# KubiakJakub01/Blokus-RL

Measured on AMD Instinct MI355X. Metric: MCTS sims/sec on 20x20 Blokus (4 players, 256 games/GPU, 100 sims/move), higher is better.
Workload: dtype fp32 net (fp32 operands split into f16 hi+lo, 3 f16 MFMA products, f32 accumulation: fp32-class error, tests/test_leafnet_gpu.py) / f64 search / u32 bitboards; 1 GPU; config 3 (N=1) / 4 (N=8): AlphaZero self-play 20x20, 256 concurrent games per GPU, 100 sims/move, ResNet-5x64 leaf eval; global_batch=256, parallelism=dp1 (independent games), model=resnet

## Files before the change

### blokus_rl_amd/csrc/mcts.hip

```cpp
#define BK_BOARD_SYNC() ::bk::wave_lds_sync()
#ifdef BK_STAMPS
#include <hip/hip_runtime.h>
static __device__ unsigned long long g_step_stamps[4096][16];
#define BK_MASK_STAMP(i) \
  do { if (threadIdx.x == 0 && blockIdx.x < 4096 && blockDim.x > 256) g_step_stamps[blockIdx.x][i] = __builtin_amdgcn_s_memtime(); } while (0)
#endif
#include <algorithm>
#include <cmath>
#include <cstring>
#include <vector>

#include "../../include/blokus_engine.h"
#include "ctx.h"
#include "legal_rows.h"
#include "mcts_dev.h"

namespace bk {

constexpr int kResetBlocks = 8;
__global__ __launch_bounds__(256) void k_reset(DevMcts m, const int32_t* flags) {
  const int t = blockIdx.y;
  if (flags && !flags[t]) return;
  TabEntry* tab = m.tab + (size_t)t * m.TS;
  for (int i = blockIdx.x * 256 + threadIdx.x; i < m.TS; i += kResetBlocks * 256) tab[i] = TabEntry{0ull, 0u, 0};
  if (blockIdx.x == 0 && threadIdx.x == 0) { m.tree_nodes[t] = 0; m.tree_children[t] = 0; }
}

constexpr int kSelectWaves = 4;
__global__ __launch_bounds__(64 * kSelectWaves) void k_select(DevPreset dp, DevMcts m, const uint32_t* __restrict__ roots,
                                                              const int32_t* __restrict__ active, double cpuct,
                                                              int32_t* __restrict__ status_out, float* __restrict__ obs,
                                                              uint64_t* __restrict__ mask_out, double root_eps, int t0) {
  extern __shared__ __attribute__((aligned(16))) uint32_t lds[];
  __shared__ int status_sh;
  const int t = t0 + blockIdx.x;
  const int wave = __builtin_amdgcn_readfirstlane(threadIdx.x >> 6);
  if (wave == 0) {
    const int st = select_descend(dp, m, t, roots, active, cpuct, status_out, lds, 0, nullptr, root_eps);
    if (lane_id() == 0) status_sh = st;
  }
  __syncthreads();
  select_leaf<kSelectWaves>(dp, m, t, status_sh, obs, mask_out, lds, wave);
}

constexpr int kLeafR = 1;
__global__ __launch_bounds__(256) void k_leaf_logits(DevPreset dp, DevMcts m, const float* __restrict__ feat,
                                                     int64_t ldf, int F, const float* __restrict__ W,
                                                     const float* __restrict__ bias) {
  extern __shared__ __attribute__((aligned(16))) uint32_t lds[];
  leaf_logits_tree<kLeafR>(dp, m, blockIdx.x, blockIdx.y, kLeafBlocks, feat, ldf, F, W, bias, lds);
}

__global__ __launch_bounds__(64) void k_expand_backup(DevPreset dp, DevMcts m, const float* __restrict__ logp,
                                                      const float* __restrict__ values, int prior_mode) {
  extern __shared__ __attribute__((aligned(16))) uint32_t lds[];
  expand_tree(dp, m, blockIdx.x, logp, values, prior_mode, lds);
}

__device__ __forceinline__ void wg_store_handoff() {
  __builtin_amdgcn_s_waitcnt(0x0F70);
  __syncthreads();
  asm volatile("buffer_inv sc0" ::: "memory");
}
constexpr int kStepWaves = 16;
__device__ __forceinline__ void leaf_zero_logits_tree(const DevPreset& dp, const DevMcts& m, int t,
                                                      const float* __restrict__ feat, int64_t ldf, int F,
                                                      uint32_t* lds) {
  const int K = leaf_logits_prologue(dp, m, t, 0, feat, ldf, F, lds);
  if (K < 0 || K > kLeafCap) return;
  const int32_t* ids = reinterpret_cast<const int32_t*>(lds + dp.W32pad);
  for (int j = threadIdx.x; j < K; j += blockDim.x) {
    m.leaf_ids[(size_t)t * kLeafCap + j] = ids[j];
    m.leaf_logit[(size_t)t * kLeafCap + j] = 0.0f;
  }
}
template <bool ROWS>
__device__ __forceinline__ void leaf_step_body(const DevPreset& dp, const DevMcts& m, const int t,
                                               const float* __restrict__ feat, int64_t ldf, int F,
                                               const float* __restrict__ W, const float* __restrict__ bias,
                                               const float* __restrict__ values, int do_select,
                                               const uint32_t* __restrict__ roots,
                                               const int32_t* __restrict__ active, double cpuct,
                                               int32_t* __restrict__ status_out, float* __restrict__ obs,
                                               uint64_t* __restrict__ mask_out, bool uninformed, int root_row) {
  extern __shared__ __attribute__((aligned(16))) uint32_t lds[];
  __shared__ int status_sh;
  const int wave = __builtin_amdgcn_readfirstlane(threadIdx.x >> 6);
#ifdef BK_STAMPS
#define BK_STEP_STAMP(i) \
  do { if (do_select && threadIdx.x == 0 && t < 4096) g_step_stamps[t][i] = __builtin_amdgcn_s_memtime(); } while (0)
#else
#define BK_STEP_STAMP(i) do { } while (0)
#endif
  BK_STEP_STAMP(0);
  if (ROWS && uninformed)
    leaf_zero_logits_tree(dp, m, t, feat, ldf, F, lds);
  else
    leaf_logits_tree<kLeafR>(dp, m, t, 0, 1, feat, ldf, F, W, bias, lds);
  wg_store_handoff();
  BK_STEP_STAMP(1);
  if (wave == 0) expand_tree<ROWS>(dp, m, t, nullptr, values, 2, lds);
  wg_store_handoff();
  BK_STEP_STAMP(2);
  if (!do_select) return;
  if (wave == 0) {
    const int st = select_descend<ROWS>(dp, m, t, roots, active, cpuct, status_out, lds, 0, nullptr, 1e-6, root_row);
    if (lane_id() == 0) status_sh = st;
  }
  __syncthreads();
  BK_STEP_STAMP(3);
  select_leaf<kStepWaves>(dp, m, t, status_sh, obs, mask_out, lds, wave);
  BK_STEP_STAMP(4);
#undef BK_STEP_STAMP
}
__global__ __launch_bounds__(64 * kStepWaves) void k_leaf_step(DevPreset dp, DevMcts m, const float* __restrict__ feat,
                                                                 int64_t ldf, int F, const float* __restrict__ W,
                                                                 const float* __restrict__ bias,
                                                                 const float* __restrict__ values, int do_select,
                                                                 const uint32_t* __restrict__ roots,
                                                                 const int32_t* __restrict__ active, double cpuct,
                                                                 int32_t* __restrict__ status_out,
                                                                 float* __restrict__ obs,
                                                                 uint64_t* __restrict__ mask_out, int t0) {
  leaf_step_body<false>(dp, m, t0 + blockIdx.x, feat, ldf, F, W, bias, values, do_select, roots, active, cpuct,
                        status_out, obs, mask_out, false, -1);
}

template <bool ROWS>
__device__ __forceinline__ void leaf_step_ov_body(const DevPreset& dp, const DevMcts& m, const int t,
                                                  const float* __restrict__ feat, int64_t ldf, int F,
                                                  const float* __restrict__ W, const float* __restrict__ bias,
                                                  const float* __restrict__ values, int do_select,
                                                  const uint32_t* __restrict__ roots,
                                                  const int32_t* __restrict__ active, double cpuct,
                                                  int32_t* __restrict__ status_out, float* __restrict__ obs,
                                                  uint64_t* __restrict__ mask_out, int sel_off, int skipz,
                                                  bool uninformed, int root_row) {
  extern __shared__ __attribute__((aligned(16))) uint32_t lds[];
  __shared__ int status_sh, status0_sh;
  __shared__ StepExpand sx;
  const int wave = __builtin_amdgcn_readfirstlane(threadIdx.x >> 6);
#ifdef BK_STAMPS
#define BK_OV_STAMP(i) \
  do { if (lane_id() == 0 && do_select && t < 4096) g_step_stamps[t][i] = __builtin_amdgcn_s_memtime(); } while (0)
#else
#define BK_OV_STAMP(i) do { } while (0)
#endif
  if (threadIdx.x == 0) {
    sx.ready = 0;
    sx.pready = 0;
    sx.done = 0;
    sx.leaf_ready = 0;
    sx.slice = 0;
    sx.loaded = 0;
    sx.counted = 0;
    sx.written = 0;
    sx.kready = 0;
    sx.hready = 0;
    status_sh = 0;
    status0_sh = m.leaf_status[t];
  }
  if (wave == 0) BK_OV_STAMP(0);
  LeafPre pre{0ull, 0.0f, false};
  if (wave > 0) pre = leaf_pre_load<kStepWaves - 1>(dp, m, t, feat, ldf, F);
  __syncthreads();
  const int status0 = status0_sh;
  int K = -1;
  if (wave > 0) {
    K = leaf_logits_prologue_w<kStepWaves - 1>(dp, m, t, feat, ldf, F, lds, wave, &sx, status0, &pre);
    if (wave == 1 && K >= 0) {
      wait_flag_acquire(&sx.hready);
      StepHead h;
      h.status = sx.hd_status;
      h.node = sx.hd_node;
      h.used = sx.hd_used;
      h.key = sx.hd_key;
      expand_head(m, t, h, K, &sx);
      BK_OV_STAMP(1);
    }
  }
  const int32_t* ids = reinterpret_cast<const int32_t*>(lds + dp.W32pad);
  float* lg = reinterpret_cast<float*>(lds + dp.W32pad + kLeafCap + F);
  uint32_t* lsel = lds + sel_off;
  uint32_t* m32 = lsel + kStateWords + 2 * kMaxN;
  if (wave == 0) {
    const StepHead h = backup_first<ROWS>(m, t, dp.P, values, status0);
    if (h.status == 1) {
      if (lane_id() == 0) {
        sx.hd_status = h.status;
        sx.hd_node = h.node;
        sx.hd_used = h.used;
        sx.hd_key = h.key;
        __hip_atomic_store(&sx.hready, 1, __ATOMIC_RELEASE, __HIP_MEMORY_SCOPE_WORKGROUP);
      }
    } else if (lane_id() == 0) {
      sx.err = -1;
      __hip_atomic_store(&sx.ready, 1, __ATOMIC_RELEASE, __HIP_MEMORY_SCOPE_WORKGROUP);
    }
    BK_OV_STAMP(2);
    if (do_select) {
      __builtin_amdgcn_s_waitcnt(0x0F70);
      asm volatile("buffer_inv sc0" ::: "memory");
      int* pend[3];
      pend[0] = &sx.ready;
      pend[1] = &sx.pready;
      pend[2] = &sx.err;
      const int st = select_descend<ROWS>(dp, m, t, roots, active, cpuct, status_out, lsel, h.key,
                                          h.status == 1 ? pend : nullptr, 1e-6, root_row);
      if (st == 1)
        for (int i = lane_id(); i < dp.W32pad / 4; i += kWave) reinterpret_cast<uint4*>(m32)[i] = make_uint4(0u, 0u, 0u, 0u);
      if (lane_id() == 0) {
        status_sh = st;
        __hip_atomic_store(&sx.leaf_ready, 1, __ATOMIC_RELEASE, __HIP_MEMORY_SCOPE_WORKGROUP);
      }
      BK_OV_STAMP(3);
      leaf_obs_rows<1>(dp, m, t, st, obs, lsel, lane_id());
    }
  }
  if (wave > 0 && K >= 0 && K <= kLeafCap) {
    if (ROWS && uninformed) {
      for (int j = (wave - 1) * kWave + lane_id(); j < K; j += (kStepWaves - 1) * kWave) lg[j] = 0.0f;
    } else {
      leaf_logits_dots<kLeafR>(dp, 0, K, wave - 1, kStepWaves - 1, W, bias, F, lds, nullptr, lg, skipz);
    }
    int done = 0;
    if (lane_id() == 0) done = __hip_atomic_fetch_add(&sx.done, 1, __ATOMIC_ACQ_REL, __HIP_MEMORY_SCOPE_WORKGROUP);
    done = readlane_i(done, 0);
    if (done == kStepWaves - 2) {
      BK_OV_STAMP(4);
      while (__hip_atomic_load(&sx.ready, __ATOMIC_ACQUIRE, __HIP_MEMORY_SCOPE_WORKGROUP) == 0)
        __builtin_amdgcn_s_sleep(1);
      const int err = readlane_i(sx.err, 0);
      if (err == 0) expand_children_lds(m, (int64_t)sx.off, K, ids, lg);
      BK_OV_STAMP(9);
      const bool descended = readlane_i(__hip_atomic_load(&sx.leaf_ready, __ATOMIC_RELAXED,
                                                          __HIP_MEMORY_SCOPE_WORKGROUP), 0) != 0;
      if (!descended) {
        __builtin_amdgcn_s_waitcnt(0x0F70);
        if (lane_id() == 0) __hip_atomic_store(&sx.pready, 1, __ATOMIC_RELEASE, __HIP_MEMORY_SCOPE_WORKGROUP);
      } else if (lane_id() == 0) {
        __hip_atomic_store(&sx.pready, 1, __ATOMIC_RELAXED, __HIP_MEMORY_SCOPE_WORKGROUP);
      }
      BK_OV_STAMP(5);
    }
  }
  if (do_select) {
    while (__hip_atomic_load(&sx.leaf_ready, __ATOMIC_ACQUIRE, __HIP_MEMORY_SCOPE_WORKGROUP) == 0)
      __builtin_amdgcn_s_sleep(1);
    if (readlane_i(status_sh, 0) == 1) mask_slices_claim(dp, lsel, m32, &sx.slice);
    if (wave == 0) BK_OV_STAMP(8);
  }
  __syncthreads();
  if (wave == 0) BK_OV_STAMP(6);
  if (!do_select) return;
  select_leaf<kStepWaves, true, false>(dp, m, t, status_sh, obs, mask_out, lsel, wave);
  if (wave == 0) BK_OV_STAMP(7);
#undef BK_OV_STAMP
}
__global__ __launch_bounds__(64 * kStepWaves) void k_leaf_step_ov(DevPreset dp, DevMcts m, const float* __restrict__ feat,
                                                                    int64_t ldf, int F, const float* __restrict__ W,
                                                                    const float* __restrict__ bias,
                                                                    const float* __restrict__ values, int do_select,
                                                                    const uint32_t* __restrict__ roots,
                                                                    const int32_t* __restrict__ active, double cpuct,
                                                                    int32_t* __restrict__ status_out,
                                                                    float* __restrict__ obs,
                                                                    uint64_t* __restrict__ mask_out, int sel_off,
                                                                    int skipz, int t0) {
  leaf_step_ov_body<false>(dp, m, t0 + blockIdx.x, feat, ldf, F, W, bias, values, do_select, roots, active, cpuct,
                           status_out, obs, mask_out, sel_off, skipz, false, -1);
}

struct RowTabs {
  const int32_t *tree, *net, *sims;
};
struct RowHeads {
  const float* W[BK_ARENA_MAX_NETS];
  const float* bias[BK_ARENA_MAX_NETS];
  int n;
};
__device__ __forceinline__ int row_live_tree(const RowTabs& rows, int r, int sim, int& budget) {
  const int t = __builtin_amdgcn_readfirstlane(rows.tree[r]);
  budget = 0;
  if (t < 0) return -1;
  budget = __builtin_amdgcn_readfirstlane(rows.sims[r]);
  return sim < budget ? t : -1;
}
__device__ __forceinline__ bool row_head(const RowTabs& rows, const RowHeads& hd, int r, const float*& W,
                                         const float*& bias, bool& uninformed) {
  const int k = __builtin_amdgcn_readfirstlane(rows.net[r]);
  uninformed = k < 0;
  W = k == 0 ? hd.W[0] : k == 1 ? hd.W[1] : k == 2 ? hd.W[2] : k == 3 ? hd.W[3] : nullptr;
  bias = k == 0 ? hd.bias[0] : k == 1 ? hd.bias[1] : k == 2 ? hd.bias[2] : k == 3 ? hd.bias[3] : nullptr;
  return k < hd.n;
}

__global__ __launch_bounds__(64 * kSelectWaves) void k_select_rows(DevPreset dp, DevMcts m, RowTabs rows,
                                                                   const uint32_t* __restrict__ roots, double cpuct,
                                                                   int32_t* __restrict__ status_out) {
  extern __shared__ __attribute__((aligned(16))) uint32_t lds[];
  __shared__ int status_sh;
  int budget;
  const int t = row_live_tree(rows, blockIdx.x, 0, budget);
  if (t < 0 || t >= m.T) return;
  const int wave = __builtin_amdgcn_readfirstlane(threadIdx.x >> 6);
  if (wave == 0) {
    const int st = select_descend<true>(dp, m, t, roots, nullptr, cpuct, status_out, lds, 0, nullptr, 1e-6, (int)blockIdx.x);
    if (lane_id() == 0) status_sh = st;
  }
  __syncthreads();
  select_leaf<kSelectWaves>(dp, m, t, status_sh, nullptr, nullptr, lds, wave);
}

__global__ __launch_bounds__(64 * kStepWaves) void k_leaf_step_rows(DevPreset dp, DevMcts m, RowTabs rows, int sim,
                                                                      const float* __restrict__ feat, int64_t ldf, int F,
                                                                      RowHeads heads, const float* __restrict__ values,
                                                                      int do_select, const uint32_t* __restrict__ roots,
                                                                      double cpuct, int32_t* __restrict__ status_out) {
  int budget;
  const int t = row_live_tree(rows, blockIdx.x, sim, budget);
  if (t < 0 || t >= m.T) return;
  const float *W, *bias;
  bool uninformed;
  if (!row_head(rows, heads, blockIdx.x, W, bias, uninformed)) return;
  leaf_step_body<true>(dp, m, t, feat, ldf, F, W, bias, uninformed ? nullptr : values,
                       do_select && sim + 1 < budget, roots, nullptr, cpuct, status_out, nullptr, nullptr, uninformed,
                       (int)blockIdx.x);
}

__global__ __launch_bounds__(64 * kStepWaves) void k_leaf_step_ov_rows(DevPreset dp, DevMcts m, RowTabs rows, int sim,
                                                                         const float* __restrict__ feat, int64_t ldf,
                                                                         int F, RowHeads heads,
                                                                         const float* __restrict__ values, int do_select,
                                                                         const uint32_t* __restrict__ roots, double cpuct,
                                                                         int32_t* __restrict__ status_out, int sel_off,
                                                                         int skipz) {
  int budget;
  const int t = row_live_tree(rows, blockIdx.x, sim, budget);
  if (t < 0 || t >= m.T) return;
  const float *W, *bias;
  bool uninformed;
  if (!row_head(rows, heads, blockIdx.x, W, bias, uninformed)) return;
  leaf_step_ov_body<true>(dp, m, t, feat, ldf, F, W, bias, uninformed ? nullptr : values,
                          do_select && sim + 1 < budget, roots, nullptr, cpuct, status_out, nullptr, nullptr, sel_off,
                          skipz, uninformed, (int)blockIdx.x);
}

__global__ __launch_bounds__(64) void k_arena_move(DevMcts m, RowTabs rows, const uint32_t* __restrict__ roots,
                                                   int32_t* __restrict__ action) {
  const int r = blockIdx.x, l = lane_id();
  const int t = __builtin_amdgcn_readfirstlane(rows.tree[r]);
  if (t < 0 || t >= m.T) {
    if (l == 0) action[r] = -1;
    return;
  }
  const uint64_t key = table_key(roots + (size_t)r * kStateWords);
  int64_t off;
  int K;
  if (!table_find(m, t, key, off, K, nullptr)) {
    if (l == 0) {
      action[r] = -1;
      atomicOr(&m.counters[kCtrErr], (unsigned long long)kErrMissingRoot);
    }
    return;
  }
  double best = -1.0;
  int bi = 0x7fffffff;
  for (int i = l; i < K; i += kWave) {
    const double v = (double)m.ch_N[off + i];
    if (v > best) { best = v; bi = i; }
  }
  wave_argmax(best, bi);
  if (l == 0) action[r] = K > 0 ? m.ch_id[off + bi] : -1;
}

__device__ __forceinline__ double raise_visits(uint32_t n, double e) {
  if (e == 1.0 || n <= 1u) return (double)n;
  return pow((double)n, e);
}

__global__ __launch_bounds__(64) void k_root(DevMcts m, const uint32_t* __restrict__ roots,
                                             const int32_t* __restrict__ active, double temperature, int mode,
                                             int32_t* ids, double* pi, uint32_t* n_out, double* q_out, float* p_out,
                                             int cap, int32_t* counts) {
  const int t = blockIdx.x;
  const int l = lane_id();
  if (active && !active[t]) {
    if (l == 0) counts[t] = 0;
    return;
  }
  const uint32_t* s = roots + (size_t)t * kStateWords;
  const uint64_t key = table_key(s);
  int64_t off;
  int K;
  if (!table_find(m, t, key, off, K, nullptr)) {
    if (l == 0) { counts[t] = -1; atomicOr(&m.counters[kCtrErr], (unsigned long long)kErrMissingRoot); }
    return;
  }
  if (l == 0) counts[t] = K <= cap ? K : -K;
  const int Kc = K <= cap ? K : cap;
  if (mode == 1) {
    for (int i = l; i < Kc; i += kWave) {
      ids[(size_t)t * cap + i] = m.ch_id[off + i];
      n_out[(size_t)t * cap + i] = m.ch_N[off + i];
      q_out[(size_t)t * cap + i] = m.ch_Q[off + i];
      p_out[(size_t)t * cap + i] = m.ch_P[off + i];
    }
    return;
  }
// ... 502 lines not shown
```

### blokus_rl_amd/csrc/mcts_dev.h

```cpp
#pragma once
#include <cmath>
#include <vector>

#include "../../include/blokus_engine.h"
#include "ctx.h"
#include "legal_rows.h"

namespace bk {

constexpr int kMaxDepth = 96;
constexpr int kExpandLdsIds = 2048;
constexpr int kGatherRegs = 16;
constexpr int kLeafCap = 2048;
constexpr int kLeafBlocks = 4;
constexpr int kMaxFeat = 2048;
constexpr int kLeafQ = 16;

#ifdef BK_STAMPS
static __device__ unsigned long long g_stamps[2][4096][8];
#define BK_STAMP(k, i) \
  do { if (lane_id() == 0 && blockIdx.x < 4096) g_stamps[k][blockIdx.x][i] = __builtin_amdgcn_s_memtime(); } while (0)
#else
#define BK_STAMP(k, i) do { } while (0)
#endif
// ... 139 lines not shown
    const double sq = sqrt((double)(uint32_t)wave_sum((int)vs) + eps);
    for (int i = l; i < K; i += kWave) {
      const double h = Q[i] + ((cp * (double)P[i]) * sq) / (1.0 + (double)Nn[i]);
      if (h > best) { best = h; bi = i; bid = ID[i]; }
    }
  }
  wave_argmax(best, bi);
  id_out = readlane_i(bid, bi & (kWave - 1));
  return bi;
}

__device__ __forceinline__ void wait_flag_acquire(int* flag) {
  while (__hip_atomic_load(flag, __ATOMIC_ACQUIRE, __HIP_MEMORY_SCOPE_WORKGROUP) == 0) __builtin_amdgcn_s_sleep(1);
  asm volatile("buffer_inv sc0" ::: "memory");
}
template <bool ROOT_ROW = false>
__device__ __forceinline__ int select_descend(const DevPreset& dp, const DevMcts& m, int t,
                                              const uint32_t* __restrict__ roots, const int32_t* __restrict__ active,
                                              double cpuct, int32_t* __restrict__ status_out, uint32_t* lds,
                                              uint64_t pend_key = 0, int* const* pend = nullptr,
                                              double root_eps = 1e-6, int root_row = -1) {
  uint32_t* s = lds;
  uint64_t* fa = reinterpret_cast<uint64_t*>(lds + kStateWords);
  const int l = lane_id();
  if (active && !active[t]) {
    if (l == 0) {
      m.leaf_status[t] = 0;
      if (status_out) status_out[t] = 0;
      m.depth[t] = 0;
    }
    return 0;
  }
  BK_STAMP(0, 0);
  load_state(s, roots + (size_t)(ROOT_ROW ? root_row : t) * kStateWords);
  BK_BOARD_SYNC();
  BK_STAMP(0, 1);
  double cp = cpuct, eps = root_eps;
  int depth = 0, err = 0;
  long long scanned = 0;
  int64_t rec_child = 0;
  int rec_pl = 0;
#ifdef BK_STAMPS
  unsigned long long t_probe = 0, t_child = 0, t_apply = 0, t_adv = 0;
#define BK_TACC(v, stmt)                                         \
  do {                                                           \
    const unsigned long long t0_ = __builtin_amdgcn_s_memtime(); \
    stmt;                                                        \
    v += __builtin_amdgcn_s_memtime() - t0_;                     \
  } while (0)
#else
#define BK_TACC(v, stmt) \
  do {                   \
    stmt;                \
  } while (0)
#endif
  for (;;) {
    int64_t off;
    int Kn;
    bool found;
    const uint64_t key = table_key(s);
    int* pend_children = nullptr;
    if (pend && key == pend_key) {
      wait_flag_acquire(pend[0]);
      if (readlane_i(*pend[2], 0) == 0) pend_children = pend[1];
      pend = nullptr;
    }
    BK_TACC(t_probe, found = table_find(m, t, key, off, Kn, nullptr));
    if (!found) break;
    if (Kn <= 0) { err |= kErrIllegal; break; }
    if (pend_children) wait_flag_acquire(pend_children);
    scanned += Kn;
    int a, ci;
    BK_TACC(t_child, ci = select_child(m, off, Kn, cp, a, eps));
    if (ci < 0 || ci >= Kn) { err |= kErrIllegal; break; }
    if (depth >= kMaxDepth) { err |= kErrDepth; break; }
    const int p = (int)s[kWToMove];
    int bad;
    BK_TACC(t_apply, bad = place_action<false>(dp, s, a, fa));
    BK_TACC(t_adv, if (!bad) advance_turn(dp, s, p, [&](int q) { return rows_any_legal(dp, s, q); }));
    if (bad) { err |= kErrIllegal; break; }
    if (depth < kWave) {
      if (l == depth) {
        rec_child = off + ci;
        rec_pl = (int)s[kWToMove];
      }
    } else if (l == 0) {
      const size_t pi = (size_t)t * kMaxDepth + depth;
      m.path_child[pi] = off + ci;
      m.path_pl[pi] = (int)s[kWToMove];
    }
    ++depth;
    cp = 1.0;
    eps = 1e-6;
  }
  if (l < depth && l < kWave) {
    const size_t pi = (size_t)t * kMaxDepth + l;
    m.path_child[pi] = rec_child;
    m.path_pl[pi] = rec_pl;
  }
  BK_STAMP(0, 2);
#ifdef BK_STAMPS
  if (lane_id() == 0 && blockIdx.x < 4096) {
    g_stamps[0][blockIdx.x][6] = t_probe;
    g_stamps[0][blockIdx.x][7] = t_child;
    g_stamps[1][blockIdx.x][7] = t_apply;
    g_stamps[1][blockIdx.x][6] = t_adv;
  }
#endif
#undef BK_TACC
  int status;
  if (err) {
    status = 0;
  } else if (s[kWFlags] & kFlagOver) {
    status = 2;
    if (l == 0) terminal_scores(dp, s, m.leaf_scores + (size_t)t * kMaxP);
  } else {
    status = 1;
  }
  if (l == 0) {
    m.leaf_status[t] = status;
    if (status_out) status_out[t] = status;
    m.depth[t] = depth;
    ctr_add(m, t, kCtrLevels, (unsigned long long)depth);
    ctr_add(m, t, kCtrScanned, (unsigned long long)scanned);
    if (status == 2) ctr_add(m, t, kCtrTerminal, 1ull);
    if (err) atomicOr(&m.counters[kCtrErr], (unsigned long long)err);
  }
  return status;
}

template <int NW>
__device__ __forceinline__ void leaf_obs_rows(const DevPreset& dp, const DevMcts& m, int t, int status,
                                              float* __restrict__ obs, const uint32_t* s, int tid) {
  if (status == 1 && tid < kWave) store_state(m.leaf_state + (size_t)t * kStateWords, s);
  const int obs_len = 2 * dp.P * dp.N * dp.N;
  float* o = obs ? obs + (size_t)t * obs_len : nullptr;
  const int tm = (int)s[kWToMove];
  const int rows = 2 * dp.P * dp.N;
  for (int pr = tid; o && pr < rows; pr += NW * kWave) {
    const int plane = pr / dp.N, r = pr - plane * dp.N;
    uint32_t bits = 0u;
    if (status == 1) bits = plane < dp.P ? s[plane * kMaxN + r] : ((plane - dp.P) == tm ? dp.full_row : 0u);
    float* dst = o + pr * dp.N;
    if ((dp.N & 3) == 0) {
      for (int c = 0; c < dp.N; c += 4)
        *reinterpret_cast<float4*>(dst + c) = make_float4((float)((bits >> c) & 1u), (float)((bits >> (c + 1)) & 1u),
                                                          (float)((bits >> (c + 2)) & 1u), (float)((bits >> (c + 3)) & 1u));
    } else {
      for (int c = 0; c < dp.N; ++c) dst[c] = (float)((bits >> c) & 1u);
    }
  }
}

template <int NW, bool BUILT = false, bool OBS = true>
__device__ __forceinline__ void select_leaf(const DevPreset& dp, const DevMcts& m, int t, int status,
                                            float* __restrict__ obs, uint64_t* __restrict__ mask_out, uint32_t* lds,
                                            int wave) {
  const uint32_t* s = lds;
  uint32_t* m32 = lds + kStateWords + 2 * kMaxN;
  const int l = lane_id(), tid = wave * kWave + l;
  const int obs_len = 2 * dp.P * dp.N * dp.N;
  if (status == 1) {
    if (BUILT)
      ;
    else if (NW == 1)
      build_mask_rows(dp, s, (int)s[kWToMove], m32);
    else
      build_mask_rows_wg<(NW > kMaskWpb ? kMaskWpb : NW)>(dp, s, (int)s[kWToMove], m32, wave);
    BK_STAMP(0, 3);
    uint64_t* mo = m.leaf_mask + (size_t)t * dp.W64;
    uint64_t* mo2 = mask_out ? mask_out + (size_t)t * dp.W64 : nullptr;
    for (int j = tid; j < dp.W64; j += NW * kWave) {
      const uint64_t w = (uint64_t)m32[2 * j] | ((uint64_t)m32[2 * j + 1] << 32);
      mo[j] = w;
      if (mo2) mo2[j] = w;
    }
    if (wave == 0 && OBS) store_state(m.leaf_state + (size_t)t * kStateWords, s);
  }
  BK_STAMP(0, 4);
  if (!OBS) return;
  float* o = obs ? obs + (size_t)t * obs_len : nullptr;
  const int tm = (int)s[kWToMove];
  const int rows = 2 * dp.P * dp.N;
  for (int pr = tid; o && pr < rows; pr += NW * kWave) {
    const int plane = pr / dp.N, r = pr - plane * dp.N;
    uint32_t bits = 0u;
    if (status == 1) bits = plane < dp.P ? s[plane * kMaxN + r] : ((plane - dp.P) == tm ? dp.full_row : 0u);
    float* dst = o + pr * dp.N;
    if ((dp.N & 3) == 0) {
      for (int c = 0; c < dp.N; c += 4)
        *reinterpret_cast<float4*>(dst + c) = make_float4((float)((bits >> c) & 1u), (float)((bits >> (c + 1)) & 1u),
                                                          (float)((bits >> (c + 2)) & 1u), (float)((bits >> (c + 3)) & 1u));
    } else {
      for (int c = 0; c < dp.N; ++c) dst[c] = (float)((bits >> c) & 1u);
    }
  }
  BK_STAMP(0, 5);
}

__device__ __forceinline__ int select_tree(const DevPreset& dp, const DevMcts& m, int t,
                                           const uint32_t* __restrict__ roots, const int32_t* __restrict__ active,
                                           double cpuct, int32_t* __restrict__ status_out, float* __restrict__ obs,
                                           uint64_t* __restrict__ mask_out, uint32_t* lds) {
  const int status = select_descend(dp, m, t, roots, active, cpuct, status_out, lds);
  select_leaf<1>(dp, m, t, status, obs, mask_out, lds, 0);
  return status;
}

__device__ __forceinline__ int leaf_logits_prologue(const DevPreset& dp, const DevMcts& m, int t, int c,
                                                    const float* __restrict__ feat, int64_t ldf, int F,
                                                    uint32_t* lds) {
  uint32_t* m32 = lds;
  int32_t* ids = reinterpret_cast<int32_t*>(lds + dp.W32pad);
  float* f = reinterpret_cast<float*>(lds + dp.W32pad + kLeafCap);
  __shared__ int Ksh;
  if (m.leaf_status[t] != 1) return -1;
  const uint64_t* lm = m.leaf_mask + (size_t)t * dp.W64;
  for (int j = threadIdx.x; j < dp.W64; j += blockDim.x) {
    const uint64_t w = lm[j];
    m32[2 * j] = (uint32_t)w;
    m32[2 * j + 1] = (uint32_t)(w >> 32);
  }
  const float* ft = feat + (size_t)t * ldf;
  for (int i = threadIdx.x; i < F; i += blockDim.x) f[i] = ft[i];
  __syncthreads();
  const int wave = threadIdx.x >> 6, l = threadIdx.x & 63;
  if (wave == 0) {
    const int K = compact_ids(dp, m32, ids, kLeafCap);
    if (l == 0) Ksh = K;
  }
  __syncthreads();
  const int K = Ksh;
  if (c == 0 && threadIdx.x == 0) {
    m.leaf_K[t] = K;
    if (K > kLeafCap) atomicOr(&m.counters[kCtrErr], (unsigned long long)kErrLeafCap);
  }
  return K;
}


__device__ __forceinline__ bool nz4(const float4& x) { return x.x != 0.f || x.y != 0.f || x.z != 0.f || x.w != 0.f; }
__device__ __forceinline__ __amdgpu_buffer_rsrc_t w_rsrc(const float* W, unsigned bytes) {
  const uintptr_t a = (uintptr_t)W;
  const uintptr_t u = ((uintptr_t)(unsigned)__builtin_amdgcn_readfirstlane((int)(a >> 32)) << 32) |
                      (unsigned)__builtin_amdgcn_readfirstlane((int)(unsigned)a);
  return __builtin_amdgcn_make_buffer_rsrc((void*)u, 0, (int)bytes, 0x00020000);
}
__device__ __forceinline__ float4 w_load(__amdgpu_buffer_rsrc_t rs, unsigned off, bool use) {
  using u32x4 = unsigned __attribute__((ext_vector_type(4)));
  const u32x4 v = __builtin_bit_cast(u32x4, __builtin_amdgcn_raw_buffer_load_b128(rs, use ? off : 0xFFFFFFF0u, 0, 0));
  return make_float4(__uint_as_float(v.x), __uint_as_float(v.y), __uint_as_float(v.z), __uint_as_float(v.w));
}
template <bool SKIP = false>
__device__ __forceinline__ float row_dot16(const float4* __restrict__ r, const float4* f4, int F4, int sub,
                                           __amdgpu_buffer_rsrc_t rs, unsigned roff) {
  float a0 = 0.f, a1 = 0.f;
  int q = sub;
  for (; q + 48 < F4; q += 64) {
    const float4 x0 = f4[q], x1 = f4[q + 16], x2 = f4[q + 32], x3 = f4[q + 48];
    float4 w0, w1, w2, w3;
    if (SKIP) {
      w0 = w_load(rs, roff + 16u * q, nz4(x0));
      w1 = w_load(rs, roff + 16u * (q + 16), nz4(x1));
      w2 = w_load(rs, roff + 16u * (q + 32), nz4(x2));
      w3 = w_load(rs, roff + 16u * (q + 48), nz4(x3));
    } else {
      w0 = r[q];
      w1 = r[q + 16];
      w2 = r[q + 32];
      w3 = r[q + 48];
    }
    a0 += w0.x * x0.x + w0.y * x0.y + w0.z * x0.z + w0.w * x0.w;
    a1 += w1.x * x1.x + w1.y * x1.y + w1.z * x1.z + w1.w * x1.w;
    a0 += w2.x * x2.x + w2.y * x2.y + w2.z * x2.z + w2.w * x2.w;
    a1 += w3.x * x3.x + w3.y * x3.y + w3.z * x3.z + w3.w * x3.w;
  }
  for (; q < F4; q += 16) {
    const float4 x0 = f4[q];
    const float4 w0 = SKIP ? w_load(rs, roff + 16u * q, nz4(x0)) : r[q];
    a0 += w0.x * x0.x + w0.y * x0.y + w0.z * x0.z + w0.w * x0.w;
  }
  float a = a0 + a1;
#pragma unroll
  for (int o = 8; o >= 1; o >>= 1) a += __shfl_xor(a, o, 16);
  return a;
}

template <int R = 1>
__device__ __forceinline__ void leaf_logits_dots(const DevPreset& dp, int lo, int hi, int wave, int nw,
                                                 const float* __restrict__ W, const float* __restrict__ bias, int F,
                                                 const uint32_t* lds, int32_t* out_ids, float* out_lg,
                                                 int skipz = 0) {
  const int32_t* ids = reinterpret_cast<const int32_t*>(lds + dp.W32pad);
  const float* f = reinterpret_cast<const float*>(lds + dp.W32pad + kLeafCap);
  const int l = threadIdx.x & 63;
  if (R > 1 && (F & 3) == 0 && F <= 64 * kLeafQ) {
    const int F4 = F >> 2;
    const float4* f4 = reinterpret_cast<const float4*>(f);
    const int sub = l & 15, quad = l >> 4;
    for (int j0 = lo + 4 * R * wave; j0 < hi; j0 += 4 * R * nw) {
      int jr[R], idr[R];
      float4 w[R][kLeafQ];
#pragma unroll
      for (int u = 0; u < R; ++u) {
        jr[u] = j0 + 4 * u + quad;
        idr[u] = ids[jr[u] < hi ? jr[u] : lo];
        const float4* r = reinterpret_cast<const float4*>(W + (size_t)idr[u] * F);
#pragma unroll
        for (int k = 0; k < kLeafQ; ++k) w[u][k] = r[sub + 16 * k < F4 ? sub + 16 * k : F4 - 1];
      }
#pragma unroll
      for (int u = 0; u < R; ++u) {
        float a0 = 0.f, a1 = 0.f;
#pragma unroll
        for (int k = 0; k < kLeafQ; ++k) {
          const int q = sub + 16 * k;
          if (q < F4) {
            const float4 x = f4[q];
            const float d = w[u][k].x * x.x + w[u][k].y * x.y + w[u][k].z * x.z + w[u][k].w * x.w;
            if ((k & 1) && sub + 16 * (k | 3) < F4)
              a1 += d;
            else
              a0 += d;
          }
        }
        float a = a0 + a1;
#pragma unroll
        for (int o = 8; o >= 1; o >>= 1) a += __shfl_xor(a, o, 16);
        if (sub == 0 && jr[u] < hi) {
          if (out_ids) out_ids[jr[u]] = idr[u];
          out_lg[jr[u]] = a + bias[idr[u]];
        }
      }
// ... 44 lines not shown
  leaf_logits_dots<R>(dp, lo, hi, (int)(threadIdx.x >> 6), (int)(blockDim.x >> 6), W, bias, F, lds,
                      m.leaf_ids + (size_t)t * kLeafCap, m.leaf_logit + (size_t)t * kLeafCap);
}

template <bool ZV = false>
__device__ __forceinline__ void expand_tree(const DevPreset& dp, const DevMcts& m, int t, const float* __restrict__ logp,
                                            const float* __restrict__ values, int prior_mode, uint32_t* lds) {
  uint32_t* m32 = lds;
  __shared__ double vsh[kMaxP];
  const int l = lane_id();
  const bool sparse = prior_mode == 2;
  const int status = m.leaf_status[t];
  const int depth = m.depth[t];
  const int node = m.tree_nodes[t];
  const int64_t used = m.tree_children[t];
  const int leafK = sparse ? m.leaf_K[t] : 0;
  const uint64_t key = table_key(m.leaf_state + (size_t)t * kStateWords);
  if (status == 0) return;
  BK_STAMP(1, 0);
  const size_t pi = (size_t)t * kMaxDepth + l;
  const bool on_path = l < depth;
  const int64_t pchild = on_path ? m.path_child[pi] : 0;
  const int ppl = on_path ? m.path_pl[pi] : 0;
  if (status == 1) {
    int err = 0;
    const int64_t room = m.child_cap_per_tree - used;
    const int64_t off = (int64_t)t * m.child_cap_per_tree + used;
    int32_t* ids_lds = reinterpret_cast<int32_t*>(m32 + dp.W32pad);
    const int cap_lds = kExpandLdsIds;
    int K;
    bool in_lds;
    BK_STAMP(1, 1);
    if (sparse) {
      K = leafK;
      in_lds = true;
      if (K > kLeafCap) err |= kErrLeafCap;
    } else {
      const uint64_t* lm = m.leaf_mask + (size_t)t * dp.W64;
      for (int j = l; j < dp.W64; j += kWave) {
        const uint64_t w = lm[j];
        m32[2 * j] = (uint32_t)w;
        m32[2 * j + 1] = (uint32_t)(w >> 32);
      }
      BK_BOARD_SYNC();
      K = compact_ids(dp, m32, ids_lds, cap_lds);
      in_lds = K <= cap_lds;
      if (!in_lds)
        K = compact_ids(dp, m32, m.ch_id + off, room > 0 ? (int)(room < 0x7fffffff ? room : 0x7fffffff) : 0);
      BK_BOARD_SYNC();
    }
    BK_STAMP(1, 2);
    if (node >= m.node_cap) err |= kErrTable;
    if (K > room) err |= kErrChildPool;
    const float* lp = sparse ? m.leaf_logit + (size_t)t * kLeafCap : logp + (size_t)t * dp.A;
    const int32_t* cid = sparse ? m.leaf_ids + (size_t)t * kLeafCap : (in_lds ? ids_lds : m.ch_id + off);
    auto logit = [&](int i) { return sparse ? lp[i] : lp[cid[i]]; };
    float x[kGatherRegs];
    int32_t xid[kGatherRegs];
#pragma unroll
    for (int j = 0; j < kGatherRegs; ++j) {
      const int i = l + j * kWave;
      const bool ok = !err && i < K;
      x[j] = ok ? logit(i) : -INFINITY;
      xid[j] = ok && in_lds ? cid[i] : 0;
    }
    int free_slot = -1;
    if (!err) {
      int64_t foff;
      int fK;
      if (table_find(m, t, key, foff, fK, &free_slot) || free_slot < 0) err |= kErrTable;
    }
    BK_STAMP(1, 3);
    if (!err) {
      float mx = -INFINITY;
#pragma unroll
      for (int j = 0; j < kGatherRegs; ++j) mx = fmaxf(mx, x[j]);
      for (int i = l + kGatherRegs * kWave; i < K; i += kWave) mx = fmaxf(mx, logit(i));
      float lse = 0.0f;
      if (prior_mode != 1) {
        mx = wave_max_f(mx);
        float sum = 0.0f;
#pragma unroll
        for (int j = 0; j < kGatherRegs; ++j) sum += l + j * kWave < K ? expf(x[j] - mx) : 0.0f;
        for (int i = l + kGatherRegs * kWave; i < K; i += kWave) sum += expf(logit(i) - mx);
        sum = wave_sum_f(sum);
        lse = logf(sum);
#pragma unroll
        for (int j = 0; j < kGatherRegs; ++j) x[j] = expf((x[j] - mx) - lse);
      }
#pragma unroll
      for (int j = 0; j < kGatherRegs; ++j) {
        const int i = l + j * kWave;
        if (i < K) {
          if (in_lds) m.ch_id[off + i] = xid[j];
          m.ch_N[off + i] = 0u;
          m.ch_Q[off + i] = 0.0;
          m.ch_P[off + i] = x[j];
        }
      }
      for (int i = l + kGatherRegs * kWave; i < K; i += kWave) {
        const float xi = logit(i);
        if (in_lds) m.ch_id[off + i] = cid[i];
        m.ch_N[off + i] = 0u;
        m.ch_Q[off + i] = 0.0;
        m.ch_P[off + i] = prior_mode != 1 ? expf((xi - mx) - lse) : xi;
      }
      if (l == 0) {
        TabEntry e;
        e.key = key;
        e.off = (uint32_t)used;
        e.K = K;
        m.tab[(size_t)t * m.TS + free_slot] = e;
        m.tree_nodes[t] = node + 1;
        m.tree_children[t] = used + K;
        ctr_add(m, t, kCtrExpanded, 1ull);
        ctr_add(m, t, kCtrLeafK, (unsigned long long)K);
      }
    } else if (l == 0) {
      atomicOr(&m.counters[kCtrErr], (unsigned long long)err);
    }
    if (l < dp.P) vsh[l] = ZV && !values ? 0.0 : (double)values[(size_t)t * dp.P + l];
  } else {
    if (l < dp.P) vsh[l] = m.leaf_scores[(size_t)t * kMaxP + l];
  }
  BK_STAMP(1, 4);
  BK_BOARD_SYNC();
  if (on_path) {
    const double v = vsh[ppl];
    const uint32_t n = m.ch_N[pchild];
    const double q = m.ch_Q[pchild];
    m.ch_Q[pchild] = ((double)n * q + v) / (double)(n + 1u);
    m.ch_N[pchild] = n + 1u;
  }
  for (int d = l + kWave; d < depth; d += kWave) {
    const size_t pd = (size_t)t * kMaxDepth + d;
    const int64_t ci = m.path_child[pd];
    const double v = vsh[m.path_pl[pd]];
    const uint32_t n = m.ch_N[ci];
    const double q = m.ch_Q[ci];
    m.ch_Q[ci] = ((double)n * q + v) / (double)(n + 1u);
    m.ch_N[ci] = n + 1u;
  }
  BK_STAMP(1, 5);
}

struct StepExpand {
  long long off;
  int K, err;
  int ready;
  int pready;
  int done;
  int leaf_ready;
  int slice;
  int loaded;
  int counted;
  int written;
  int kready;
  int hready;
  int wcnt[16];
  int hd_status, hd_node;
  long long hd_used;
  unsigned long long hd_key;
};

struct StepHead {
  int status, node;
  int64_t used;
  uint64_t key;
};
template <bool ZV = false>
__device__ __forceinline__ StepHead backup_first(const DevMcts& m, int t, int P, const float* __restrict__ values,
                                                 int status) {
  __shared__ double vsh[kMaxP];
  const int l = lane_id();
  StepHead h;
  h.status = status;
  const int depth = m.depth[t];
  h.node = m.tree_nodes[t];
  h.used = m.tree_children[t];
  h.key = table_key(m.leaf_state + (size_t)t * kStateWords);
  if (h.status == 0) return h;
  const size_t pi = (size_t)t * kMaxDepth + l;
  const bool on_path = l < depth;
  const int64_t pchild = on_path ? m.path_child[pi] : 0;
  const int ppl = on_path ? m.path_pl[pi] : 0;
  if (h.status == 1) {
    if (l < P) vsh[l] = ZV && !values ? 0.0 : (double)values[(size_t)t * P + l];
  } else {
    if (l < P) vsh[l] = m.leaf_scores[(size_t)t * kMaxP + l];
  }
  wave_lds_sync();
  if (on_path) {
    const double v = vsh[ppl];
    const uint32_t n = m.ch_N[pchild];
    const double q = m.ch_Q[pchild];
    m.ch_Q[pchild] = ((double)n * q + v) / (double)(n + 1u);
    m.ch_N[pchild] = n + 1u;
  }
  for (int d = l + kWave; d < depth; d += kWave) {
    const size_t pd = (size_t)t * kMaxDepth + d;
    const int64_t ci = m.path_child[pd];
    const double v = vsh[m.path_pl[pd]];
    const uint32_t n = m.ch_N[ci];
    const double q = m.ch_Q[ci];
    m.ch_Q[ci] = ((double)n * q + v) / (double)(n + 1u);
    m.ch_N[ci] = n + 1u;
  }
  return h;
}

__device__ __forceinline__ void expand_head(const DevMcts& m, int t, const StepHead& h, int K, StepExpand* sx) {
  const int l = lane_id();
  int err = 0;
  if (h.status == 1) {
    const int64_t room = m.child_cap_per_tree - h.used;
    if (K > kLeafCap) err |= kErrLeafCap;
    if (h.node >= m.node_cap) err |= kErrTable;
    if (K > room) err |= kErrChildPool;
    int free_slot = -1;
    if (!err) {
      int64_t foff;
      int fK;
      if (table_find(m, t, h.key, foff, fK, &free_slot) || free_slot < 0) err |= kErrTable;
    }
    if (!err) {
      if (l == 0) {
        TabEntry e;
        e.key = h.key;
        e.off = (uint32_t)h.used;
        e.K = K;
        m.tab[(size_t)t * m.TS + free_slot] = e;
        m.tree_nodes[t] = h.node + 1;
        m.tree_children[t] = h.used + K;
        ctr_add(m, t, kCtrExpanded, 1ull);
        ctr_add(m, t, kCtrLeafK, (unsigned long long)K);
      }
    } else if (l == 0) {
      atomicOr(&m.counters[kCtrErr], (unsigned long long)err);
    }
  }
  __builtin_amdgcn_s_waitcnt(0x0F70);
  if (l == 0) {
    sx->off = (long long)((int64_t)t * m.child_cap_per_tree + h.used);
    sx->K = K;
    sx->err = h.status == 1 ? err : -1;
    __hip_atomic_store(&sx->ready, 1, __ATOMIC_RELEASE, __HIP_MEMORY_SCOPE_WORKGROUP);
  }
}

struct LeafPre {
  uint64_t w;
  float f;
  bool ok;
};
template <int NW>
__device__ __forceinline__ LeafPre leaf_pre_load(const DevPreset& dp, const DevMcts& m, int t,
                                                 const float* __restrict__ feat, int64_t ldf, int F) {
  const int tid = threadIdx.x - kWave, nth = NW * kWave;
  LeafPre p;
  p.ok = dp.W64 <= nth && F <= nth;
  p.w = p.ok && tid < dp.W64 ? m.leaf_mask[(size_t)t * dp.W64 + tid] : 0ull;
  p.f = p.ok && tid < F ? feat[(size_t)t * ldf + tid] : 0.0f;
  return p;
}
template <int NW>
__device__ __forceinline__ int leaf_logits_prologue_w(const DevPreset& dp, const DevMcts& m, int t,
                                                      const float* __restrict__ feat, int64_t ldf, int F,
                                                      uint32_t* lds, int wave, StepExpand* sx, int status,
                                                      const LeafPre* pre = nullptr) {
  uint32_t* m32 = lds;
  int32_t* ids = reinterpret_cast<int32_t*>(lds + dp.W32pad);
  float* f = reinterpret_cast<float*>(lds + dp.W32pad + kLeafCap);
  if (status != 1) return -1;
  const int tid = threadIdx.x - kWave, nth = NW * kWave, l = lane_id();
  if (pre && pre->ok) {
    if (tid < dp.W64) {
      m32[2 * tid] = (uint32_t)pre->w;
      m32[2 * tid + 1] = (uint32_t)(pre->w >> 32);
    }
    if (tid < F) f[tid] = pre->f;
  } else {
    const uint64_t* lm = m.leaf_mask + (size_t)t * dp.W64;
    for (int j = tid; j < dp.W64; j += nth) {
      const uint64_t w = lm[j];
      m32[2 * j] = (uint32_t)w;
      m32[2 * j + 1] = (uint32_t)(w >> 32);
    }
    const float* ft = feat + (size_t)t * ldf;
    for (int i = tid; i < F; i += nth) f[i] = ft[i];
  }
  auto arrive_wait = [&](int* ctr) {
    if (l == 0) __hip_atomic_fetch_add(ctr, 1, __ATOMIC_ACQ_REL, __HIP_MEMORY_SCOPE_WORKGROUP);
    while (__hip_atomic_load(ctr, __ATOMIC_ACQUIRE, __HIP_MEMORY_SCOPE_WORKGROUP) < NW) __builtin_amdgcn_s_sleep(1);
  };
  arrive_wait(&sx->loaded);
  const int w = 64 * (wave - 1) + l;
  uint32_t bits = w < dp.W32 ? m32[w] : 0u;
  const int cnt = __popc(bits);
  const int incl = wave_incl_scan(cnt);
  if (l == kWave - 1) sx->wcnt[wave] = incl;
  arrive_wait(&sx->counted);
  int before = 0, K = 0;
  for (int v = 1; v <= NW; ++v) {
    const int c = sx->wcnt[v];
    before += v < wave ? c : 0;
    K += c;
  }
  int pos = before + incl - cnt;
  while (bits) {
    const int b = __ffs(bits) - 1;
    bits &= bits - 1u;
    if (pos < kLeafCap) ids[pos] = w * 32 + b;
    ++pos;
  }
  arrive_wait(&sx->written);
  if (wave == 1 && l == 0) {
    m.leaf_K[t] = K;
    if (K > kLeafCap) atomicOr(&m.counters[kCtrErr], (unsigned long long)kErrLeafCap);
    __hip_atomic_store(&sx->kready, K + 1, __ATOMIC_RELEASE, __HIP_MEMORY_SCOPE_WORKGROUP);
  }
  return K;
}

#ifdef BK_STAMPS
static __device__ unsigned long long g_mask_stamps[256][16][6];
#endif
__device__ __forceinline__ void mask_slices_claim(const DevPreset& dp, const uint32_t* s, uint32_t* m32, int* counter) {
#ifdef BK_STAMPS
  const unsigned long long t_in = __builtin_amdgcn_s_memtime();
  unsigned long long n_cl = 0, t_max = 0, t_first_claim = 0;
  int last_k = -1;
#endif
  RowCtx c = row_ctx(dp, s, (int)s[kWToMove], m32);
  for (;;) {
#ifdef BK_STAMPS
    const unsigned long long t_s = __builtin_amdgcn_s_memtime();
    if (t_first_claim == 0) t_first_claim = t_s;
#endif
#pragma unroll
    for (int d = 0; d < 5; ++d) asm volatile("" : "+v"(c.fr[d]), "+v"(c.ar[d]));
    asm volatile("" : "+v"(c.r), "+v"(c.rN1), "+v"(c.pieces));
    int k = 0;
    if (lane_id() == 0) k = __hip_atomic_fetch_add(counter, 1, __ATOMIC_RELAXED, __HIP_MEMORY_SCOPE_WORKGROUP);
    k = readlane_i(k, 0);
    if (k >= kMaskWpb) break;
    DevPreset dq = dp;
    asm volatile("" : "+s"(dq.N), "+s"(dq.num_pieces));
    orient_dispatch<kMaskWpb>(dq, c, k, std::make_index_sequence<kMaskWpb>{});
#ifdef BK_STAMPS
    ++n_cl;
    last_k = k;
    const unsigned long long d = __builtin_amdgcn_s_memtime() - t_s;
    t_max = d > t_max ? d : t_max;
#endif
  }
#ifdef BK_STAMPS
  const unsigned long long t_out = __builtin_amdgcn_s_memtime();
  unsigned long long t_warm = 0;
  if (last_k >= 0) {
    DevPreset dq = dp;
    asm volatile("" : "+s"(dq.N), "+s"(dq.num_pieces));
    const unsigned long long t0 = __builtin_amdgcn_s_memtime();
    orient_dispatch<kMaskWpb>(dq, c, last_k, std::make_index_sequence<kMaskWpb>{});
    t_warm = __builtin_amdgcn_s_memtime() - t0;
  }
  const int w = (int)(threadIdx.x >> 6);
  if (lane_id() == 0 && blockIdx.x < 256 && w < 16) {
    g_mask_stamps[blockIdx.x][w][0] = t_in;
    g_mask_stamps[blockIdx.x][w][1] = n_cl;
    g_mask_stamps[blockIdx.x][w][2] = t_out;
    g_mask_stamps[blockIdx.x][w][3] = t_max;
    g_mask_stamps[blockIdx.x][w][4] = t_warm;
    g_mask_stamps[blockIdx.x][w][5] = t_first_claim;
  }
#endif
}

__device__ __forceinline__ void expand_children_lds(const DevMcts& m, int64_t off, int K, const int32_t* ids,
                                                    const float* lg) {
  const int l = lane_id();
  float x[kGatherRegs];
  int32_t xid[kGatherRegs];
#pragma unroll
  for (int j = 0; j < kGatherRegs; ++j) {
    const int i = l + j * kWave;
    const bool ok = i < K;
    x[j] = ok ? lg[i] : -INFINITY;
    xid[j] = ok ? ids[i] : 0;
  }
  float mx = -INFINITY;
#pragma unroll
  for (int j = 0; j < kGatherRegs; ++j) mx = fmaxf(mx, x[j]);
  for (int i = l + kGatherRegs * kWave; i < K; i += kWave) mx = fmaxf(mx, lg[i]);
  mx = wave_max_f(mx);
  float sum = 0.0f;
#pragma unroll
  for (int j = 0; j < kGatherRegs; ++j) sum += l + j * kWave < K ? expf(x[j] - mx) : 0.0f;
  for (int i = l + kGatherRegs * kWave; i < K; i += kWave) sum += expf(lg[i] - mx);
  sum = wave_sum_f(sum);
  const float lse = logf(sum);
#pragma unroll
  for (int j = 0; j < kGatherRegs; ++j) x[j] = expf((x[j] - mx) - lse);
#pragma unroll
  for (int j = 0; j < kGatherRegs; ++j) {
    const int i = l + j * kWave;
    if (i < K) {
      m.ch_id[off + i] = xid[j];
      m.ch_N[off + i] = 0u;
      m.ch_Q[off + i] = 0.0;
      m.ch_P[off + i] = x[j];
    }
  }
  for (int i = l + kGatherRegs * kWave; i < K; i += kWave) {
    m.ch_id[off + i] = ids[i];
    m.ch_N[off + i] = 0u;
    m.ch_Q[off + i] = 0.0;
    m.ch_P[off + i] = expf((lg[i] - mx) - lse);
  }
}

}

struct bk_mcts {
  bk_ctx* ctx = nullptr;
  bk::DevMcts d{};
  std::vector<void*> allocs;
  static constexpr int kMaxGroups = 4;
  bool pipe_ready = false;
  hipStream_t pipe_stream[kMaxGroups - 1] = {};
  hipEvent_t pipe_fork = nullptr, pipe_step[kMaxGroups] = {}, pipe_join[kMaxGroups - 1] = {};
};
```

Measured before the change: 1.404 million sims/s.

## Replace end-of-step barrier with last-builder wave storing the leaf mask

Drops the final workgroup barrier and the cooperative select_leaf mask store in the overlapped leaf-step kernel. Each wave that builds a mask slice bumps a shared counter, and the wave that finishes the last slice waits on kready and writes the mask to global memory by itself. Waves also skip building the row context when no slice is left to claim. Other waves can exit without waiting on the slowest one, but the store now runs on a single wave, and the BUILT/OBS template paths are removed.

```diff
diff --git a/blokus_rl_amd/csrc/mcts.hip b/blokus_rl_amd/csrc/mcts.hip
--- a/blokus_rl_amd/csrc/mcts.hip
+++ b/blokus_rl_amd/csrc/mcts.hip
@@ -152,6 +152,10 @@
     sx.done = 0;
     sx.leaf_ready = 0;
     sx.slice = 0;
+    sx.built = 0;
+#ifdef BK_STAMPS
+    sx.exited = 0;
+#endif
     sx.loaded = 0;
     sx.counted = 0;
     sx.written = 0;
@@ -247,14 +251,20 @@
   if (do_select) {
     while (__hip_atomic_load(&sx.leaf_ready, __ATOMIC_ACQUIRE, __HIP_MEMORY_SCOPE_WORKGROUP) == 0)
       __builtin_amdgcn_s_sleep(1);
-    if (readlane_i(status_sh, 0) == 1) mask_slices_claim(dp, lsel, m32, &sx.slice);
+    if (readlane_i(status_sh, 0) == 1 && mask_slices_claim(dp, lsel, m32, &sx.slice, &sx.built)) {
+      if (status0 == 1) wait_flag_acquire(&sx.kready);
+      leaf_mask_store(dp, m, t, m32, mask_out);
+      BK_OV_STAMP(6);
+    }
     if (wave == 0) BK_OV_STAMP(8);
   }
-  __syncthreads();
-  if (wave == 0) BK_OV_STAMP(6);
-  if (!do_select) return;
-  select_leaf<kStepWaves, true, false>(dp, m, t, status_sh, obs, mask_out, lsel, wave);
-  if (wave == 0) BK_OV_STAMP(7);
+#ifdef BK_STAMPS
+  {
+    int n = 0;
+    if (lane_id() == 0) n = __hip_atomic_fetch_add(&sx.exited, 1, __ATOMIC_RELAXED, __HIP_MEMORY_SCOPE_WORKGROUP);
+    if (readlane_i(n, 0) == kStepWaves - 1) BK_OV_STAMP(7);
+  }
+#endif
 #undef BK_OV_STAMP
 }
 __global__ __launch_bounds__(64 * kStepWaves) void k_leaf_step_ov(DevPreset dp, DevMcts m, const float* __restrict__ feat,
diff --git a/blokus_rl_amd/csrc/mcts_dev.h b/blokus_rl_amd/csrc/mcts_dev.h
--- a/blokus_rl_amd/csrc/mcts_dev.h
+++ b/blokus_rl_amd/csrc/mcts_dev.h
@@ -315,7 +315,7 @@
   }
 }
 
-template <int NW, bool BUILT = false, bool OBS = true>
+template <int NW>
 __device__ __forceinline__ void select_leaf(const DevPreset& dp, const DevMcts& m, int t, int status,
                                             float* __restrict__ obs, uint64_t* __restrict__ mask_out, uint32_t* lds,
                                             int wave) {
@@ -324,9 +324,7 @@
   const int l = lane_id(), tid = wave * kWave + l;
   const int obs_len = 2 * dp.P * dp.N * dp.N;
   if (status == 1) {
-    if (BUILT)
-      ;
-    else if (NW == 1)
+    if (NW == 1)
       build_mask_rows(dp, s, (int)s[kWToMove], m32);
     else
       build_mask_rows_wg<(NW > kMaskWpb ? kMaskWpb : NW)>(dp, s, (int)s[kWToMove], m32, wave);
@@ -338,10 +336,9 @@
       mo[j] = w;
       if (mo2) mo2[j] = w;
     }
-    if (wave == 0 && OBS) store_state(m.leaf_state + (size_t)t * kStateWords, s);
+    if (wave == 0) store_state(m.leaf_state + (size_t)t * kStateWords, s);
   }
   BK_STAMP(0, 4);
-  if (!OBS) return;
   float* o = obs ? obs + (size_t)t * obs_len : nullptr;
   const int tm = (int)s[kWToMove];
   const int rows = 2 * dp.P * dp.N;
@@ -692,6 +689,10 @@
   int done;
   int leaf_ready;
   int slice;
+  int built;
+#ifdef BK_STAMPS
+  int exited;
+#endif
   int loaded;
   int counted;
   int written;
@@ -865,39 +866,51 @@
 #ifdef BK_STAMPS
 static __device__ unsigned long long g_mask_stamps[256][16][6];
 #endif
-__device__ __forceinline__ void mask_slices_claim(const DevPreset& dp, const uint32_t* s, uint32_t* m32, int* counter) {
+__device__ __forceinline__ bool mask_slices_claim(const DevPreset& dp, const uint32_t* s, uint32_t* m32, int* counter,
+                                                  int* built) {
 #ifdef BK_STAMPS
   const unsigned long long t_in = __builtin_amdgcn_s_memtime();
-  unsigned long long n_cl = 0, t_max = 0, t_first_claim = 0;
+  unsigned long long n_cl = 0, t_max = 0, t_ctx = t_in, t_warm = 0;
   int last_k = -1;
 #endif
-  RowCtx c = row_ctx(dp, s, (int)s[kWToMove], m32);
-  for (;;) {
-#ifdef BK_STAMPS
-    const unsigned long long t_s = __builtin_amdgcn_s_memtime();
-    if (t_first_claim == 0) t_first_claim = t_s;
-#endif
-#pragma unroll
-    for (int d = 0; d < 5; ++d) asm volatile("" : "+v"(c.fr[d]), "+v"(c.ar[d]));
-    asm volatile("" : "+v"(c.r), "+v"(c.rN1), "+v"(c.pieces));
+  auto claim = [&]() {
     int k = 0;
     if (lane_id() == 0) k = __hip_atomic_fetch_add(counter, 1, __ATOMIC_RELAXED, __HIP_MEMORY_SCOPE_WORKGROUP);
-    k = readlane_i(k, 0);
-    if (k >= kMaskWpb) break;
-    DevPreset dq = dp;
-    asm volatile("" : "+s"(dq.N), "+s"(dq.num_pieces));
-    orient_dispatch<kMaskWpb>(dq, c, k, std::make_index_sequence<kMaskWpb>{});
+    return readlane_i(k, 0);
+  };
+  bool last = false;
+  int k = claim();
+  if (k < kMaskWpb) {
+    RowCtx c = row_ctx(dp, s, (int)s[kWToMove], m32);
 #ifdef BK_STAMPS
-    ++n_cl;
-    last_k = k;
-    const unsigned long long d = __builtin_amdgcn_s_memtime() - t_s;
-    t_max = d > t_max ? d : t_max;
+    t_ctx = __builtin_amdgcn_s_memtime();
 #endif
+    do {
+#ifdef BK_STAMPS
+      const unsigned long long t_s = __builtin_amdgcn_s_memtime();
+#endif
+#pragma unroll
+      for (int d = 0; d < 5; ++d) asm volatile("" : "+v"(c.fr[d]), "+v"(c.ar[d]));
+      asm volatile("" : "+v"(c.r), "+v"(c.rN1), "+v"(c.pieces));
+      DevPreset dq = dp;
+      asm volatile("" : "+s"(dq.N), "+s"(dq.num_pieces));
+      orient_dispatch<kMaskWpb>(dq, c, k, std::make_index_sequence<kMaskWpb>{});
+      int b = 0;
+      if (lane_id() == 0) b = __hip_atomic_fetch_add(built, 1, __ATOMIC_ACQ_REL, __HIP_MEMORY_SCOPE_WORKGROUP);
+      last = readlane_i(b, 0) == kMaskWpb - 1;
+#ifdef BK_STAMPS
+      ++n_cl;
+      last_k = k;
+      const unsigned long long d = __builtin_amdgcn_s_memtime() - t_s;
+      t_max = d > t_max ? d : t_max;
+#endif
+      k = claim();
+    } while (k < kMaskWpb);
   }
 #ifdef BK_STAMPS
   const unsigned long long t_out = __builtin_amdgcn_s_memtime();
-  unsigned long long t_warm = 0;
-  if (last_k >= 0) {
+  if (last_k >= 0 && !last) {
+    RowCtx c = row_ctx(dp, s, (int)s[kWToMove], m32);
     DevPreset dq = dp;
     asm volatile("" : "+s"(dq.N), "+s"(dq.num_pieces));
     const unsigned long long t0 = __builtin_amdgcn_s_memtime();
@@ -911,9 +924,21 @@
     g_mask_stamps[blockIdx.x][w][2] = t_out;
     g_mask_stamps[blockIdx.x][w][3] = t_max;
     g_mask_stamps[blockIdx.x][w][4] = t_warm;
-    g_mask_stamps[blockIdx.x][w][5] = t_first_claim;
+    g_mask_stamps[blockIdx.x][w][5] = t_ctx;
   }
 #endif
+  return last;
+}
+
+__device__ __forceinline__ void leaf_mask_store(const DevPreset& dp, const DevMcts& m, int t, const uint32_t* m32,
+                                                uint64_t* __restrict__ mask_out) {
+  uint64_t* mo = m.leaf_mask + (size_t)t * dp.W64;
+  uint64_t* mo2 = mask_out ? mask_out + (size_t)t * dp.W64 : nullptr;
+  for (int j = lane_id(); j < dp.W64; j += kWave) {
+    const uint64_t w = (uint64_t)m32[2 * j] | ((uint64_t)m32[2 * j + 1] << 32);
+    mo[j] = w;
+    if (mo2) mo2[j] = w;
+  }
 }
 
 __device__ __forceinline__ void expand_children_lds(const DevMcts& m, int64_t off, int K, const int32_t* ids,
```

Result: no change. 1.406 million sims/s (median of 6 runs) (+0.2%).
